# bioinformatics-centre/kaiju

Measured on AMD Instinct MI355X. Metric: classified reads/sec (150 bp), higher is better.
Workload: dtype u64

## Files before the change

kaiju_amd/csrc/capi.hip:

```cpp
#include <hip/hip_runtime.h>
#include <fcntl.h>
#include <sys/stat.h>
#include <time.h>
#include <unistd.h>

#include <algorithm>
#include <atomic>
#include <cstdio>
#include <cstring>
#include <future>
#include <memory>
#include <mutex>
#include <stdexcept>
#include <string>
#include <thread>
#include <vector>
#include <chrono>

#include "../../include/kaiju_gpu.h"
#include "fmi_stream.h"
#include "host_index.h"
#include "host_tables.h"
#include "kj_core.h"
#include "taxonomy.h"
// ... 203 lines not shown
  {
    const bool td = need || later;
    const uint64_t m = __ballot(td);
    if (m) {
      const uint32_t leader = (uint32_t)__builtin_ctzll(m);
      uint32_t base = 0;
      if (lane == leader) base = atomicAdd(todocount, (uint32_t)__popcll(m));
      base = (uint32_t)__shfl((int)base, (int)leader, 64);
      if (td) todo[base + (uint32_t)__popcll(m & ((1ull << lane) - 1ull))] = r;
    }
  }
}
template <bool LCA>
__global__ void __launch_bounds__(256)
k_mem_post2(DevIndex ix, Params p, Batch b, DevTaxonomy t, CompactHit *__restrict__ compact, const uint32_t *__restrict__ todo,
            const uint32_t *__restrict__ todocount) {
  const uint32_t n = *todocount;
  for (uint32_t i = blockIdx.x * 256 + threadIdx.x; i < n; i += gridDim.x * 256) {
    const uint32_t r = todo[i];
    Hit *h = b.hits + r;
    if (!mem_locate_read<false>(ix, p, h, kLocDeferRows)) mem_locate_read<false, true>(ix, p, h);
    if (LCA) compact[r] = compact_hit(t, *h);
  }
}

__global__ void __launch_bounds__(kFragBlock)
k_fragments_protein(const ConstTables *__restrict__ g_ct, Params p, SegTables st, Batch b, SegQueue sq, uint32_t *err) {
  __shared__ ConstTables s_ct;
  __shared__ int32_t s_entg[17];
  __shared__ uint8_t s_code[256];
  if (threadIdx.x < 17) s_entg[threadIdx.x] = st.ent_g32[threadIdx.x];
  {
    const uint32_t *src = reinterpret_cast<const uint32_t *>(g_ct);
    uint32_t *dst = reinterpret_cast<uint32_t *>(&s_ct);
    for (uint32_t i = threadIdx.x; i < sizeof(ConstTables) / 4; i += kFragBlock) dst[i] = src[i];
    for (uint32_t i = threadIdx.x; i < 256; i += kFragBlock) s_code[i] = 0;
    __syncthreads();
    if (threadIdx.x < 20) protein_code_entry(s_ct, threadIdx.x, s_code);
    __syncthreads();
  }
  const uint32_t r = blockIdx.x * kFragBlock + threadIdx.x;
  if (r >= b.n_reads) return;
  uint32_t e = 0;
  build_fragments_protein(s_ct, s_code, p, TrigCtx{s_entg, st.ent_locut32}, b, sq, r, &e);
  if (e) atomicOr(err, e);
}

struct CoopWave {
  uint64_t *prefix = nullptr;
  __device__ __forceinline__ uint64_t *pref() const { return prefix; }
  __device__ __forceinline__ void sync() const { __syncthreads(); }
  __device__ __forceinline__ int lane() const { return (int)(threadIdx.x & 63u); }
  __device__ __forceinline__ int width() const { return 64; }
  __device__ __forceinline__ void reduce_min(double &prob, int &t) const {
#pragma unroll
    for (int o = 32; o > 0; o >>= 1) {
      const double op = __shfl_xor(prob, o, 64);
      const int ot = __shfl_xor(t, o, 64);
      if (op < prob || (op == prob && ot < t)) { prob = op; t = ot; }
    }
  }
};

template <int T>
struct CoopTeam {
  uint64_t *prefix = nullptr;
  __device__ __forceinline__ uint64_t *pref() const { return prefix; }
  __device__ __forceinline__ void sync() const { __builtin_amdgcn_fence(__ATOMIC_ACQ_REL, "workgroup"); __builtin_amdgcn_wave_barrier(); }
  __device__ __forceinline__ int lane() const { return (int)(threadIdx.x & (uint32_t)(T - 1)); }
  __device__ __forceinline__ int width() const { return T; }
  __device__ __forceinline__ void reduce_min(double &prob, int &t) const {
#pragma unroll
    for (int o = T / 2; o > 0; o >>= 1) {
      const double op = __shfl_xor(prob, o, 64);
      const int ot = __shfl_xor(t, o, 64);
      if (op < prob || (op == prob && ot < t)) { prob = op; t = ot; }
    }
  }
};

constexpr int kSegBlock = 64, kSegStage = 2048;
__global__ void __launch_bounds__(kSegBlock)
k_seg(Params p, SegTables st, Batch b, SegQueue sq) {
  __shared__ int64_t s_entg[13];
  __shared__ double s_lnf[kSegLnf];
  __shared__ __attribute__((aligned(16))) uint8_t s_frag[kSegStage];
  __shared__ int32_t s_work[4 * kSegMaxRegions];
  __shared__ uint8_t s_cls[kSegStage];
  if (threadIdx.x < 13) s_entg[threadIdx.x] = st.ent_g[threadIdx.x];
  if (threadIdx.x < kSegLnf) s_lnf[threadIdx.x] = st.lnfact[threadIdx.x];
  __syncthreads();
  const SegCtx cx = seg_ctx(st, s_entg, s_lnf);
  __shared__ uint64_t s_pref[2 * (kSegPacked + 1)];
  CoopWave coop;
  coop.prefix = s_pref;
  const uint32_t n = min(*sq.count, sq.cap);
  for (uint32_t s = blockIdx.x; s < n; s += gridDim.x)
    seg_compute(cx, coop, b, p, sq, s, s_frag, kSegStage, s_work, s_cls, [] { __syncthreads(); });
}
#ifndef KJ_SEG_WAVES
#define KJ_SEG_WAVES 3
#endif
template <int T>
__global__ void __launch_bounds__(kSegBlock, KJ_SEG_WAVES)
k_seg_teams(Params p, SegTables st, Batch b, SegQueue sq) {
  constexpr int NT = kSegBlock / T, kStage = kSegStage / NT;
  __shared__ int64_t s_entg[13];
  __shared__ double s_lnf[kSegLnf];
  __shared__ __attribute__((aligned(16))) uint8_t s_frag[kSegStage];
  __shared__ int32_t s_work[NT * 4 * kSegMaxRegions];
  __shared__ uint8_t s_cls[kSegStage];
  if (threadIdx.x < 13) s_entg[threadIdx.x] = st.ent_g[threadIdx.x];
  if (threadIdx.x < kSegLnf) s_lnf[threadIdx.x] = st.lnfact[threadIdx.x];
  __syncthreads();
  const SegCtx cx = seg_ctx(st, s_entg, s_lnf);
  __shared__ uint64_t s_pref[NT * 2 * (kSegPacked + 1)];
  const uint32_t team = threadIdx.x / (uint32_t)T;
  CoopTeam<T> coop;
  coop.prefix = s_pref + team * 2 * (kSegPacked + 1);
  const uint32_t n = min(*sq.count, sq.cap);
  for (uint32_t s0 = blockIdx.x * NT; s0 < n; s0 += gridDim.x * NT) {
    const uint32_t s = s0 + team;
    if (s < n)
      seg_compute(cx, coop, b, p, sq, s, s_frag + team * kStage, kStage, s_work + team * 4 * kSegMaxRegions, s_cls + team * kStage,
                  [] { __builtin_amdgcn_fence(__ATOMIC_ACQ_REL, "workgroup"); __builtin_amdgcn_wave_barrier(); });
  }
}

__global__ void __launch_bounds__(kBlock)
k_seg_apply(const ConstTables *__restrict__ g_ct, Params p, Batch b, SegQueue sq, uint32_t *err) {
  __shared__ ConstTables s_ct;
  load_tables(s_ct, g_ct);
  const uint32_t r = blockIdx.x * kBlock + threadIdx.x;
  if (r >= b.n_reads) return;
  uint32_t e = 0;
  seg_apply_mem(s_ct, p, b, sq, r, &e);
  if (e) atomicOr(err, e);
}

template <class P>
__device__ __forceinline__ void mem_body(const DevIndex &ix, const Params &p, const Batch &b, const WorkList &wl,
                                         SIEntry *si_all, uint32_t si_cap, const VerboseOut &vb) {
  __shared__ __attribute__((aligned(16))) uint8_t s_win[kBlock * kWinStride];
  const uint64_t lane = (uint64_t)blockIdx.x * kBlock + threadIdx.x;
  LaneScratch ls;
  ls.si = si_all + lane * si_cap;
  ls.si_cap = si_cap;
  ls.win = s_win + threadIdx.x * kWinStride;
  mem_lane<P>(ix, p, b, wl, ls, vb);
}
#ifndef KJ_MEM_WAVES
#define KJ_MEM_WAVES 4
#endif
#ifdef KJ_PROF
__global__ void __launch_bounds__(kBlock, 3)
#else
__global__ void __launch_bounds__(kBlock, KJ_MEM_WAVES)
#endif
k_mem(DevIndex ix, Params p, Batch b, WorkList wl, SIEntry *si_all, uint32_t si_cap) {
  __shared__ __attribute__((aligned(16))) uint8_t s_win[kBlock * kWinStride];
  const uint64_t lane = (uint64_t)blockIdx.x * kBlock + threadIdx.x;
  LaneScratch ls;
  ls.si = si_all + lane * si_cap;
  ls.si_cap = si_cap;
  ls.win = s_win + threadIdx.x * kWinStride;
#ifdef KJ_PROF
  __shared__ unsigned long long s_prof[kBlock / 64][2 + 3 * PM_N];
  for (int x = threadIdx.x & 63; x < 2 + 3 * PM_N; x += 64) s_prof[threadIdx.x >> 6][x] = 0;
  ls.prof = s_prof[threadIdx.x >> 6];
  if ((threadIdx.x & 63) == 0) { ls.prof[0] = __builtin_readcyclecounter(); ls.prof[1] = PM_HEAD; }
#endif
  mem_lane2<false>(ix, p, b, wl, ls);
}
template <bool WIDE>
__global__ void __launch_bounds__(256)
k_mem_locate(DevIndex ix, Params p, Batch b, uint32_t *list, uint32_t *count) {
  const uint32_t r = blockIdx.x * 256 + threadIdx.x;
  const bool defer = r < b.n_reads && !mem_locate_read<WIDE>(ix, p, b.hits + r, list ? kLocDeferRows : 0u);
  const uint64_t m = __ballot(defer);
// ... 1292 lines not shown
  KJ_HIP(hipMemcpy(host_out, static_cast<const uint8_t *>(a.p) + offset_bytes, n_bytes, hipMemcpyDeviceToHost));
  return KAIJU_GPU_OK;
  });
}

struct kaiju_gpu_taxonomy {
  int device = 0;
  DevTaxonomy dev{};
  std::vector<void *> allocs;
  ~kaiju_gpu_taxonomy() {
    (void)hipSetDevice(device);
    for (void *p : allocs) (void)hipFree(p);
  }
};

__global__ void __launch_bounds__(256)
k_lca(DevTaxonomy t, const Hit *__restrict__ hits, uint32_t n, CompactHit *__restrict__ out) {
  const uint32_t r = blockIdx.x * 256 + threadIdx.x;
  if (r >= n) return;
  out[r] = compact_hit(t, hits[r]);
}

struct DevBuf {
  void *p = nullptr;
  size_t cap = 0;
};

struct kaiju_gpu_ctx {
  const kaiju_gpu_index *ix = nullptr;
  kaiju_gpu_params params{};
  Params kp{};
  hipStream_t stream = nullptr;
  hipEvent_t ev[6] = {nullptr, nullptr, nullptr, nullptr, nullptr, nullptr};
  bool ev_valid = false;
  int n_cu = 0, blocks_main = 0, blocks_retry = 0;
  DevBuf pep, frags, meta, counters, retry_list, seg_items, seg_recs;
  DevBuf scratch_main[10], scratch_retry[5], h_compact;
  DevBuf redo_bitmap, redo_list, redo_items, redo_index, redo_pool, redo_work, redo_cls;
  bool greedy2 = false;
  bool greedy3 = false;
  uint32_t g3_split = 1;
  uint32_t g3_threads = 512;
  uint32_t g1_pool = 192, g1_match = 64;
  bool g1_pool_set = false;
  uint32_t greedy_gate = 1u | 32u << 8;
  bool verbose = false;
  bool exact_pass = true;
  bool count_ops = false;
  bool mem_v1 = false;
  bool verbose_v1 = false;
  bool stage1_old = false;
  bool stage1_lane = false;
  bool lazy_seg = true;
  DevBuf seglist, loc_list, todo_list;
  int seg_team = 64;
  bool fused_post = true;
  const char *dump_frags = nullptr;
  uint32_t vb_text_cap = 0;
  DevBuf vb_nacc, vb_acc, vb_tlen, vb_text, vb_bestv, vb_bestv_retry;
  DevBuf vb_packed, vb_pos;
  std::vector<uint8_t> vb_host;
  std::vector<uint32_t> vb_h_nacc, vb_h_acc;
  DevBuf h_seqs, h_off, h_hits;
  kj_ingest_scratch *ingest = nullptr;
  DevBuf ing_text1, ing_text2, ing_names, ing_info;
  kj_format_scratch *format = nullptr;
  DevBuf fmt_pw, fmt_out, fmt_info;
  bool fmt_pw_ok = false;
  kaiju_gpu_stats stats{};
  uint32_t last_n = 0;
  uint32_t max_read_len = 1024;
  ~kaiju_gpu_ctx() {
    if (!ix) return;
    (void)hipSetDevice(ix->device);
    if (ingest) kj_ingest_free(ingest);
    if (format && kj_format_free) kj_format_free(format);
    DevBuf *all[] = {&fmt_pw, &fmt_out, &fmt_info, &ing_text1, &ing_text2, &ing_names, &ing_info, &pep, &frags, &meta, &counters, &retry_list, &seg_items, &seg_recs, &h_seqs, &h_off, &h_hits, &h_compact, &seglist, &loc_list, &todo_list,
                     &vb_nacc, &vb_acc, &vb_tlen, &vb_text, &vb_bestv, &vb_bestv_retry, &vb_packed, &vb_pos,
                     &redo_bitmap, &redo_list, &redo_items, &redo_index, &redo_pool, &redo_work, &redo_cls};
    for (DevBuf *b : all) if (b->p) (void)hipFree(b->p);
    for (int i = 0; i < 10; i++) if (scratch_main[i].p) (void)hipFree(scratch_main[i].p);
    for (int i = 0; i < 5; i++) if (scratch_retry[i].p) (void)hipFree(scratch_retry[i].p);
    for (auto &e : ev) if (e) (void)hipEventDestroy(e);
    if (stream) (void)hipStreamDestroy(stream);
  }
};

static int ensure(DevBuf &b, size_t bytes) {
  if (bytes <= b.cap) return 0;
  if (b.p) { KJ_HIP(hipFree(b.p)); b.p = nullptr; b.cap = 0; }
  const size_t want = bytes + bytes / 8 + 256;
  KJ_HIP(hipMalloc(&b.p, want));
  b.cap = want;
  return 0;
}

extern "C" void kaiju_gpu_default_params(kaiju_gpu_params *p, int mode) {
  if (!p) return;
  p->mode = mode ? 1 : 0;
  p->min_fragment_length = 11;
  p->mismatches = 3;
  p->min_score = 65;
  p->seed_length = 7;
  p->seg = 1;
  p->use_evalue = mode ? 1 : 0;
  p->min_evalue = 0.01;
  p->max_matches_SI = 20;
  p->max_match_ids = 20;
  p->input_is_protein = 0;
}

extern "C" int kaiju_gpu_create(kaiju_gpu_ctx **out, const kaiju_gpu_index *ix, const kaiju_gpu_params *p) {
  return guarded([&]() -> int {
  if (!out || !ix || !p) return fail(KAIJU_GPU_ERR_ARG, "NULL argument");
  *out = nullptr;
  if (p->mode != 0 && p->mode != 1) return fail(KAIJU_GPU_ERR_ARG, "mode must be 0 (MEM) or 1 (GREEDY)");
  if (p->min_fragment_length < 1 || p->min_fragment_length > 10000)
    return fail(KAIJU_GPU_ERR_UNSUPPORTED, "min_fragment_length out of range");
  if (p->mode == 1 && p->mismatches > (uint32_t)kMaxMismatch)
    return fail(KAIJU_GPU_ERR_UNSUPPORTED, "more than 8 mismatches are not supported");
  if (p->mode == 1 && p->seed_length < 1) return fail(KAIJU_GPU_ERR_ARG, "seed_length must be >= 1");
  if (p->max_match_ids > 20 || p->max_matches_SI > 64 || p->max_matches_SI < 1)
    return fail(KAIJU_GPU_ERR_UNSUPPORTED, "max_match_ids <= 20 and 1 <= max_matches_SI <= 64 required");
  std::unique_ptr<kaiju_gpu_ctx> c(new kaiju_gpu_ctx());
  c->ix = ix;
  c->params = *p;
  c->kp.mode = p->mode; c->kp.m = p->min_fragment_length; c->kp.mismatches = p->mismatches;
  c->kp.min_score = p->min_score; c->kp.seed_length = p->seed_length; c->kp.seg = p->seg ? 1 : 0;
  c->kp.max_matches_SI = p->max_matches_SI; c->kp.max_match_ids = p->max_match_ids;
  if (const char *e = getenv("KAIJU_GPU_DEBUG")) c->kp.debug = (uint32_t)atoi(e);
  if (const char *e = getenv("KAIJU_GPU_EXACT_PASS")) c->exact_pass = atoi(e) != 0;
  if (const char *e = getenv("KAIJU_GPU_MEM_LANE")) c->mem_v1 = !strcmp(e, "v1");
  if (const char *e = getenv("KAIJU_GPU_VERBOSE_LANE")) c->verbose_v1 = !strcmp(e, "v1");
  c->dump_frags = getenv("KAIJU_GPU_DUMP_FRAGS");
  if (const char *e = getenv("KAIJU_GPU_STAGE1")) { c->stage1_old = !strcmp(e, "old"); c->stage1_lane = !strcmp(e, "lane"); }
  if (const char *e = getenv("KAIJU_GPU_LAZY_SEG")) c->lazy_seg = atoi(e) != 0;
  if (const char *e = getenv("KAIJU_GPU_FUSED_POST")) c->fused_post = atoi(e) != 0;
  if (const char *e = getenv("KAIJU_GPU_SEG_TEAM")) { const int v = atoi(e); if (v == 8 || v == 16 || v == 32 || v == 64) c->seg_team = v; }
  if (ix->id_mode == KAIJU_GPU_IDS_SEQUENCE && p->mode == 0) c->kp.flags |= kParamXOrder;
  if (p->input_is_protein) c->kp.flags |= kParamProtein;
  KJ_HIP(hipSetDevice(ix->device));
  hipDeviceProp_t prop;
  KJ_HIP(hipGetDeviceProperties(&prop, ix->device));
  c->n_cu = prop.multiProcessorCount;
  int occ = 0;
  if (p->mode == 0) KJ_HIP(hipOccupancyMaxActiveBlocksPerMultiprocessor(&occ, k_mem, kBlock, 0));
  else {
    const bool g_wide = ix->dev.mb_base != nullptr;
    const uint32_t g_k = g_wide ? ix->dev.kmer_k : ix->dev.kline_k;
    c->greedy2 = ix->dev.blocks64 && (g_wide ? ix->dev.kmer64 != nullptr : ix->dev.kline != nullptr) && g_k >= 2 &&
                 g_k <= p->seed_length && p->seed_length >= 3;
    if (const char *e = getenv("KAIJU_GPU_GREEDY_LANE")) { if (!strcmp(e, "v1")) c->greedy2 = false; }
#ifdef KJ_GREEDY3
    if (const char *e = getenv("KAIJU_GPU_GREEDY_LANE")) { if (!strcmp(e, "v3")) c->greedy3 = c->greedy2 && !g_wide; }
    if (const char *e = getenv("KAIJU_GPU_G3_SPLIT")) c->g3_split = (uint32_t)atoi(e);
    if (const char *e = getenv("KAIJU_GPU_G3_THREADS")) { const int v = atoi(e); if (v >= 64 && v <= kG3Threads && v % 64 == 0) c->g3_threads = (uint32_t)v; }
#else
    if (const char *e = getenv("KAIJU_GPU_GREEDY_LANE")) {
      if (!strcmp(e, "v3")) return fail(KAIJU_GPU_ERR_UNSUPPORTED, "KAIJU_GPU_GREEDY_LANE=v3: this library was built without -DKJ_GREEDY3 (tests/tools/mem_variants.sh, variant g3)");
    }
#endif
    if (const char *e = getenv("KAIJU_GPU_GREEDY_GATE")) { int v = atoi(e); if (v == 0 || v == 1 || v == 3 || v == 7 || v == 15) c->greedy_gate = (c->greedy_gate & ~0xffu) | (uint32_t)v; }
    if (const char *e = getenv("KAIJU_GPU_GREEDY_WAITERS")) { int v = atoi(e); if (v >= 0 && v <= 64) c->greedy_gate = (c->greedy_gate & 0xffu) | (uint32_t)v << 8; }
    if (c->greedy2) {
      KJ_HIP(hipFuncSetAttribute(reinterpret_cast<const void *>(k_greedy2), hipFuncAttributeMaxDynamicSharedMemorySize,
                                 (int)kGreedy2Lds));
      KJ_HIP(hipFuncSetAttribute(reinterpret_cast<const void *>(k_greedy2_count), hipFuncAttributeMaxDynamicSharedMemorySize,
                                 (int)kGreedy2Lds));
      KJ_HIP(hipFuncSetAttribute(reinterpret_cast<const void *>(k_greedy2_wide), hipFuncAttributeMaxDynamicSharedMemorySize,
                                 (int)kGreedy2Lds));
      KJ_HIP(hipFuncSetAttribute(reinterpret_cast<const void *>(k_greedy2_wide_count), hipFuncAttributeMaxDynamicSharedMemorySize,
                                 (int)kGreedy2Lds));
      KJ_HIP(hipFuncSetAttribute(reinterpret_cast<const void *>(k_greedy2_vb), hipFuncAttributeMaxDynamicSharedMemorySize, (int)kGreedy2Lds));
      KJ_HIP(hipFuncSetAttribute(reinterpret_cast<const void *>(k_greedy2_wide_vb), hipFuncAttributeMaxDynamicSharedMemorySize, (int)kGreedy2Lds));
      if (g_wide) KJ_HIP(hipOccupancyMaxActiveBlocksPerMultiprocessor(&occ, k_greedy2_wide, kBlock, kGreedy2Lds));
      else KJ_HIP(hipOccupancyMaxActiveBlocksPerMultiprocessor(&occ, k_greedy2, kBlock, kGreedy2Lds));
    } else KJ_HIP(hipOccupancyMaxActiveBlocksPerMultiprocessor(&occ, k_greedy, kBlock, 0));
  }
  if (occ < 1) occ = 1;
  if (occ > 8) occ = 8;
  if (const char *e = getenv("KAIJU_GPU_BLOCKS_PER_CU")) { int v = atoi(e); if (v >= 1 && v <= 8) occ = v; }
  c->blocks_main = c->n_cu * occ;
  c->blocks_retry = p->mode == 0 ? 16 : 4;
  if (const char *e = getenv("KAIJU_GPU_G1_POOL")) { int v = atoi(e); if (v >= 64 && v <= 65535) { c->g1_pool = (uint32_t)v; c->g1_pool_set = true; } }
  if (const char *e = getenv("KAIJU_GPU_G1_MATCH")) { int v = atoi(e); if (v >= 16 && v <= 65535) c->g1_match = (uint32_t)v; }
  if (const char *e = getenv("KAIJU_GPU_RETRY_BLOCKS")) { int v = atoi(e); if (v >= 1 && v <= 256) c->blocks_retry = v; }
  KJ_HIP(hipStreamCreateWithFlags(&c->stream, hipStreamNonBlocking));
  for (auto &e : c->ev) KJ_HIP(hipEventCreate(&e));
  {
// ... 167 lines not shown
    if ((rc = ensure(c->scratch_main[0], lanes_main * si_cap * sizeof(SIEntry)))) return rc;
    const uint32_t si_cap_retry = (uint32_t)std::min<uint64_t>(2 * max_pair + 64, 1u << 24);
    int blocks_retry = c->blocks_retry;
    while (blocks_retry > 1 && (uint64_t)blocks_retry * kBlock * si_cap_retry * sizeof(SIEntry) > (1ull << 30)) blocks_retry /= 2;
    if ((rc = ensure(c->scratch_retry[0], (uint64_t)blocks_retry * kBlock * si_cap_retry * sizeof(SIEntry)))) return rc;
    if (n > 0) {
      const bool xo = (p.flags & kParamXOrder) != 0;
      SIEntry *si_main = static_cast<SIEntry *>(c->scratch_main[0].p);
      auto launch_v2 = [&](const Params &pp, const WorkList &wl, bool counting, bool second = false) {
        if (c->verbose) {
          if (mem_narrow2) hipLaunchKernelGGL(k_mem_vb, dim3(c->blocks_main), blk, 0, s, ix->dev, pp, b, wl, si_main, si_cap, vb.acc);
          else hipLaunchKernelGGL(k_mem_wide2_vb, dim3(c->blocks_main), blk, 0, s, ix->dev, pp, b, wl, si_main, si_cap, vb.acc);
        } else
        if (mem_narrow2) {
          if (second && !xo) hipLaunchKernelGGL(k_mem_second, dim3(c->blocks_main), blk, 0, s, ix->dev, pp, b, wl, si_main, si_cap);
          else if (counting) hipLaunchKernelGGL(k_mem_count, dim3(c->blocks_main), blk, 0, s, ix->dev, pp, b, wl, si_main, si_cap);
          else if (xo) hipLaunchKernelGGL(k_mem_x, dim3(c->blocks_main), blk, 0, s, ix->dev, pp, b, wl, si_main, si_cap);
          else hipLaunchKernelGGL(k_mem, dim3(c->blocks_main), blk, 0, s, ix->dev, pp, b, wl, si_main, si_cap);
        } else {
          if (counting) hipLaunchKernelGGL(k_mem_wide2_count, dim3(c->blocks_main), blk, 0, s, ix->dev, pp, b, wl, si_main, si_cap);
          else if (xo) hipLaunchKernelGGL(k_mem_wide2_x, dim3(c->blocks_main), blk, 0, s, ix->dev, pp, b, wl, si_main, si_cap);
          else hipLaunchKernelGGL(k_mem_wide2, dim3(c->blocks_main), blk, 0, s, ix->dev, pp, b, wl, si_main, si_cap);
        }
      };
      const bool defer = mem_v2;
      Params pd = p;
      if (defer) pd.flags |= kParamDeferLocate;
      if (mem_v2) {
        Params pm = pd;
        if (lazy) pm.flags |= kParamLazySeg;
        launch_v2(pm, wl_main, c->count_ops);
      } else if (!ix->dev.mb_base)
        hipLaunchKernelGGL(k_mem_v1, dim3(c->blocks_main), blk, 0, s, ix->dev, p, b, wl_main, si_main, si_cap, vb);
      else
        hipLaunchKernelGGL(k_mem_wide, dim3(c->blocks_main), blk, 0, s, ix->dev, p, b, wl_main, si_main, si_cap, vb);
      KJ_HIP(hipGetLastError());
      KJ_HIP(hipEventRecord(c->ev[3], s));
      uint32_t *todo = nullptr;
      const DevTaxonomy dt = tax ? tax->dev : DevTaxonomy{};
      CompactHit *const cmp = reinterpret_cast<CompactHit *>(d_compact);
      if (fused) {
        if ((rc = ensure(c->seglist, (size_t)n * 4 + 16))) return rc;
        if ((rc = ensure(c->todo_list, (size_t)n * 4 + 16))) return rc;
        todo = static_cast<uint32_t *>(c->todo_list.p);
        uint32_t *seglist = static_cast<uint32_t *>(c->seglist.p);
        if (tax) hipLaunchKernelGGL(k_mem_post1<true>, grid_reads, dim3(256), 0, s, ix->d_s1, ix->dev, p, b, dt, cmp, lazy ? 1 : 0, seglist, cnt + 22, todo, cnt + 26);
        else hipLaunchKernelGGL(k_mem_post1<false>, grid_reads, dim3(256), 0, s, ix->d_s1, ix->dev, p, b, dt, cmp, lazy ? 1 : 0, seglist, cnt + 22, todo, cnt + 26);
        KJ_HIP(hipGetLastError());
      }
      if (lazy) {
        if ((rc = ensure(c->seglist, (size_t)n * 4 + 16))) return rc;
        uint32_t *seglist = static_cast<uint32_t *>(c->seglist.p);
        if (!fused) hipLaunchKernelGGL(k_trigcheck, grid_reads, dim3(256), 0, s, ix->d_s1, p, b, seglist, cnt + 22);
        hipLaunchKernelGGL(k_segflag, dim3(c->n_cu * 4), dim3(256), 0, s, p, ix->st, b, sq, seglist, cnt + 22, cnt + 3);
        launch_seg(c, s, p, ix->st, b, sq);
        hipLaunchKernelGGL(k_seg_apply_list, dim3(c->n_cu * 4), blk, 0, s, ix->d_ct, p, b, sq, seglist, cnt + 22, cnt + 3);
        WorkList wl_seg;
        wl_seg.counter = cnt + 23; wl_seg.reads = seglist; wl_seg.n_items_ptr = cnt + 22; wl_seg.n_items = 0;
        wl_seg.retry_list = wl_main.retry_list; wl_seg.retry_count = wl_main.retry_count;
        launch_v2(pd, wl_seg, false, true);
        KJ_HIP(hipGetLastError());
      }
      hipLaunchKernelGGL(k_mem_retry, dim3(blocks_retry), blk, 0, s, ix->dev, p, b, wl_retry,
                         static_cast<SIEntry *>(c->scratch_retry[0].p), si_cap_retry, vb);
      KJ_HIP(hipGetLastError());
      if (defer && c->verbose) {
        if (mem_narrow2) hipLaunchKernelGGL(k_mem_verbose<false>, grid_reads, dim3(256), 0, s, ix->dev, p, b, vb);
        else hipLaunchKernelGGL(k_mem_verbose<true>, grid_reads, dim3(256), 0, s, ix->dev, p, b, vb);
        KJ_HIP(hipGetLastError());
      }
      if (defer && !fused) {
        if (mem_narrow2 && ix->dev.row_tax) {
          hipLaunchKernelGGL(k_mem_locate<false>, grid_reads, dim3(256), 0, s, ix->dev, p, b, loc_list, cnt + 24);
          hipLaunchKernelGGL(k_mem_locate_list<false>, dim3(c->n_cu * 8), dim3(256), 0, s, ix->dev, p, b, loc_list, cnt + 24);
        }
        else if (mem_narrow2) hipLaunchKernelGGL(k_mem_locate_team, grid_team, dim3(256), 0, s, ix->dev, p, b);
        else if (ix->dev.row_tax) {
          hipLaunchKernelGGL(k_mem_locate<true>, grid_reads, dim3(256), 0, s, ix->dev, p, b, loc_list, cnt + 24);
          hipLaunchKernelGGL(k_mem_locate_list<true>, dim3(c->n_cu * 8), dim3(256), 0, s, ix->dev, p, b, loc_list, cnt + 24);
        }
        else hipLaunchKernelGGL(k_mem_locate_wide, grid_team, dim3(256), 0, s, ix->dev, p, b);
        KJ_HIP(hipGetLastError());
      }
      if (exact_pass) {
        xp.si = static_cast<SIEntry *>(c->scratch_retry[0].p); xp.si_cap = si_cap_retry; xp.blocks_search = blocks_retry;
        xp.vb = vb;
        KJ_HIP(kj_launch_exact_pass(xp));
      }
      if (fused) {
        if (tax) hipLaunchKernelGGL(k_mem_post2<true>, dim3(c->n_cu * 8), dim3(256), 0, s, ix->dev, p, b, dt, cmp, todo, cnt + 26);
        else hipLaunchKernelGGL(k_mem_post2<false>, dim3(c->n_cu * 8), dim3(256), 0, s, ix->dev, p, b, dt, cmp, todo, cnt + 26);
        KJ_HIP(hipGetLastError());
      }
    } else KJ_HIP(hipEventRecord(c->ev[3], s));
  } else {
    const uint32_t frag_max = max_read_len / 3 + 4;
    GreedyArrays ga;
    ga.pool_cap = (c->verbose && !c->g1_pool_set) ? std::max<uint32_t>(c->g1_pool, 512u) : c->g1_pool; ga.match_cap = c->g1_match;
    const bool vb_g2 = c->verbose && !c->verbose_v1 && max_read_len / 3 + 4 < 65536;
    const bool use_g2 = c->greedy2 && (!c->verbose || vb_g2);
    const bool use_g3 = use_g2 && c->greedy3 && !c->verbose;
#ifdef KJ_GREEDY3
    const uint64_t lanes_g2 = use_g3 ? (uint64_t)c->n_cu * kG3Pool : lanes_main;
#else
    const uint64_t lanes_g2 = lanes_main;
#endif
    if (!use_g2) {
      if ((rc = ensure(c->scratch_main[0], lanes_main * ga.pool_cap * sizeof(GItem)))) return rc;
      if ((rc = ensure(c->scratch_main[1], lanes_main * ga.pool_cap * sizeof(uint16_t)))) return rc;
// ... 838 lines not shown
```

kaiju_amd/csrc/kj_core.h:

```cpp
#pragma once
#include <type_traits>
#include <stdint.h>

#if defined(__HIPCC__)
#include <hip/hip_runtime.h>
#define KJ_HD __host__ __device__ __forceinline__
#define KJ_HD_NOINLINE __host__ __device__ __noinline__
#else
#define KJ_HD inline
#define KJ_HD_NOINLINE inline
struct uint2 { uint32_t x, y; };
struct ulonglong2 { uint64_t x, y; };
#endif

namespace kj {

struct u128 { uint64_t x, y; };
typedef u128 u128_unaligned __attribute__((aligned(1)));
typedef uint32_t u32_unaligned __attribute__((aligned(1)));
typedef uint64_t u64_unaligned __attribute__((aligned(1)));

constexpr int kMaxIds = 21;
constexpr int kSbShift = 16;
constexpr uint32_t kHitIdCap = 1u, kHitSiCap = 2u;
// ... 373 lines not shown
  for (uint64_t step = 0; step <= n; step++) {
    if (tpos5 && (k & tvm) == 0) put_tpos5(tpos5, k >> tv_shift, g);
    if (row_tax) row_tax[k] = dense;
    const uint32_t c = symbol_at(ix, k);
    if (text) text[g - 1] = (uint8_t)c;
    if (c == 0) return;
    k = rank_c(ix, c, k);
    g--;
  }
}

KJ_HD uint32_t kmer_index(uint32_t idx, uint32_t c) { return idx * 20u + (c - 1u); }
KJ_HD void kmer_lookup(const DevIndex &ix, uint32_t idx, uint64_t &lo, uint64_t &hi) {
  if (ix.kmer32) { const uint2 e = ix.kmer32[idx]; lo = e.x; hi = (uint64_t)e.x + e.y; }
  else { const ulonglong2 e = ix.kmer64[idx]; lo = e.x; hi = e.x + e.y; }
}

KJ_HD uint32_t codon_fwd(const ConstTables &t, const uint8_t *s) {
  const uint32_t a = t.nuc[s[0]], b = t.nuc[s[1]], c = t.nuc[s[2]];
  if ((a | b | c) > 3u) return 255u;
  return t.codon_aa[a * 16 + b * 4 + c];
}
KJ_HD uint32_t codon_rev(const ConstTables &t, const uint8_t *s) {
  const uint32_t a = t.nuc[s[2]], b = t.nuc[s[1]], c = t.nuc[s[0]];
  if ((a | b | c) > 3u) return 255u;
  return t.codon_aa[(3 - a) * 16 + (3 - b) * 4 + (3 - c)];
}

constexpr int kSegWindow = 12, kSegDown = 5, kSegUp = 7, kSegMaxTrim = 50;
constexpr int kSegMaxRegions = 32;
constexpr int kSegPacked = 63;
constexpr int kSegLnf = 64;

#define KJ_SL(s, i) ((uint32_t)(s)[(i)] - 1u)

struct SegCtx {
  const int64_t *ent_g;
  int64_t ent_locut, ent_hicut;
  const double *lnf;
  const double *lnfact;
  uint32_t lnfact_n;
};
KJ_HD SegCtx seg_ctx(const SegTables &st, const int64_t *ent_g, const double *lnf) {
  SegCtx c; c.ent_g = ent_g; c.ent_locut = st.ent_locut; c.ent_hicut = st.ent_hicut;
  c.lnf = lnf; c.lnfact = st.lnfact; c.lnfact_n = st.lnfact_n;
  return c;
}

struct CoopSerial {
  uint64_t *prefix = nullptr;
  KJ_HD int lane() const { return 0; }
  KJ_HD int width() const { return 1; }
  KJ_HD void reduce_min(double &, int &) const {}
  KJ_HD uint64_t *pref() const { return prefix; }
  KJ_HD void sync() const {}
};

struct SegWin {
  uint64_t c0, c1;
  int64_t score;
};
KJ_HD void segwin_add(SegWin &w, const SegCtx &cx, uint32_t a, int d) {
  const uint32_t old = a < 16 ? (uint32_t)(w.c0 >> (4 * a)) & 15u : (uint32_t)(w.c1 >> (4 * (a - 16))) & 15u;
  w.score += cx.ent_g[(int)old + d] - cx.ent_g[old];
  if (a < 16) w.c0 += (uint64_t)(int64_t)d << (4 * a);
  else w.c1 += (uint64_t)(int64_t)d << (4 * (a - 16));
}
template <class S>
KJ_HD void segwin_open(SegWin &w, const SegCtx &cx, const S &s, int start) {
  w.c0 = w.c1 = 0; w.score = 0;
  for (int i = 0; i < kSegWindow; i++) segwin_add(w, cx, KJ_SL(s, start + i), +1);
}
template <class S>
KJ_HD void segwin_shift(SegWin &w, const SegCtx &cx, const S &s, int start) {
  segwin_add(w, cx, KJ_SL(s, start), -1);
  segwin_add(w, cx, KJ_SL(s, start + kSegWindow), +1);
}

KJ_HD double kj_lnfact(const SegCtx &cx, int n) {
  if (n < kSegLnf) return cx.lnf[n];
  return cx.lnfact[(uint32_t)n < cx.lnfact_n ? n : cx.lnfact_n - 1];
}

KJ_HD double seg_finish_prob(double ans1, double ans2, int total) {
  const double totseq = ((double)total) * 2.9957322735539909;
#if defined(__HIP_DEVICE_COMPILE__)
  return __dsub_rn(__dadd_rn(ans1, ans2), totseq);
#else
  volatile double t = ans1 + ans2;
  return t - totseq;
#endif
}

KJ_HD int zero_fields6(uint64_t x) {
  const uint64_t LOW5 = 0x7DF7DF7DF7DF7DFull;
  const uint64_t HI = 0x820820820820820ull;
  const uint64_t nzmask = (((x & LOW5) + LOW5) | x) & HI;
  return 10 - (int)popc64(nzmask);
}

KJ_HD double seg_prob_of_counts(const SegCtx &cx, uint64_t c0, uint64_t c1, int l);
KJ_HD double seg_window_prob_packed(const SegCtx &cx, const uint8_t *s, int l, int i) {
  uint64_t c0 = 0, c1 = 0;
  for (int k = 0; k < l; k++) {
    const uint32_t a = KJ_SL(s, i + k);
    if (a < 10) c0 += 1ull << (6 * a); else c1 += 1ull << (6 * (a - 10));
// ... 117 lines not shown
      while (loi - 1 >= lowlim && (cls[loi - 1 - first] & 2)) loi--;
      while (hii + 1 <= last && (cls[hii + 1 - first] & 2)) hii++;
    } else {
      if (wi + 1 == i) segwin_shift(w, cx, s, wi - first);
      else if (wi != i) segwin_open(w, cx, s, i - first);
      wi = i;
      if (w.score > cx.ent_locut) continue;
      {
        SegWin b;
        while (loi - 1 >= lowlim) {
          segwin_open(b, cx, s, loi - 1 - first);
          if (b.score > cx.ent_hicut) break;
          loi--;
        }
      }
      {
        SegWin f = w;
        while (hii + 1 <= last) {
          segwin_shift(f, cx, s, hii - first);
          if (f.score > cx.ent_hicut) break;
          hii++;
        }
      }
    }
    const int rawleft = loi - kSegDown, rawright = hii + kSegUp - 1;
    int tl, tr;
    seg_trim(cx, coop, s + rawleft, rawright - rawleft + 1, tl, tr);
    const int leftend = rawleft + tl, rightend = rawleft + tr;
    if constexpr (TOP) {
      if (i + kSegUp - 1 < leftend) {
        int32_t tb[1], te[1];
        bool ov = false;
        const int k = seg_scan<false>(cx, coop, s + rawleft, leftend - rawleft, offset + rawleft, tb, te, 0, 1, ov,
                                      cls ? cls + rawleft : nullptr);
        if (k > 0) {
          if (n < cap) { beg[n] = tb[0]; end[n] = te[0]; n++; } else overflow = true;
        }
      }
    }
    if constexpr (TOP) {
      if (n < cap) { beg[n] = leftend + offset; end[n] = rightend + offset; n++; } else overflow = true;
    } else {
      beg[0] = leftend + offset; end[0] = rightend + offset; n = 1;
    }
    i = hii < rightend + kSegDown ? hii : rightend + kSegDown;
    lowlim = i + 1;
  }
  return n;
}

template <class Coop, class Sync>
KJ_HD int seg_regions(const SegCtx &cx, const Coop &coop, const uint8_t *s, int len,
                      int32_t *left, int32_t *right, bool &overflow, int32_t *work, uint8_t *cls, Sync &&team_sync,
                      int cap = kSegMaxRegions) {
  int32_t *b = work, *e = work + cap;
  if (cls && len >= kSegWindow) {
    seg_classes(cx, coop, s, len, cls);
    team_sync();
  }
  const int n = seg_scan<true>(cx, coop, s, len, 0, b, e, 0, cap, overflow, cls);
  if (n == 0) return 0;
  int m = 0;
  int32_t cb = b[n - 1], ce = e[n - 1];
  for (int k = n - 2; k >= 0; k--) {
    if (cb - e[k] - 1 < 0) {
      if (ce < e[k]) ce = e[k];
      if (cb > b[k]) cb = b[k];
    } else {
      left[m] = cb; right[m] = ce; m++;
      cb = b[k]; ce = e[k];
    }
  }
  left[m] = cb; right[m] = ce; m++;
  for (int a = 0, z = m - 1; a < z; a++, z--) {
    int32_t t = left[a]; left[a] = left[z]; left[z] = t;
    t = right[a]; right[a] = right[z]; right[z] = t;
  }
  return m;
}

#if defined(__HIP_DEVICE_COMPILE__)
KJ_HD uint32_t fetch_work(uint32_t *counter) { return atomicAdd(counter, 1u); }
KJ_HD uint32_t append_slot(uint32_t *counter) { return atomicAdd(counter, 1u); }
#else
KJ_HD uint32_t fetch_work(uint32_t *counter) { return (*counter)++; }
KJ_HD uint32_t append_slot(uint32_t *counter) { return (*counter)++; }
#endif

struct PepBuf {
  uint8_t *base;
  uint32_t row;
  KJ_HD uint8_t get(uint32_t p) const { return base[(size_t)(p >> 2) * row + (p & 3u)]; }
  KJ_HD void put(uint32_t p, uint8_t v) const { base[(size_t)(p >> 2) * row + (p & 3u)] = v; }
  KJ_HD uint32_t get32(uint32_t p) const { return *reinterpret_cast<const uint32_t *>(base + (size_t)(p >> 2) * row); }
};
struct PepView {
  PepBuf b;
  uint32_t off;
  KJ_HD uint8_t operator[](int i) const { return b.get(off + (uint32_t)i); }
};

template <class S>
KJ_HD uint32_t diag_score(const ConstTables &t, const S &pep, uint32_t start, uint32_t len) {
  uint32_t s = 0;
  for (uint32_t i = 0; i < len; i++) { const uint32_t a = t.idx_to_aa[pep[start + i]]; s += (uint32_t)t.b62[a][a]; }
  return s;
}

KJ_HD void frag_insert(Frag *list, uint32_t &n, uint32_t cap, const Frag &f) {
// ... 206 lines not shown
    src = stage;
  }
  int32_t *left = work + 2 * kSegMaxRegions, *right = work + 3 * kSegMaxRegions;
  bool ov = false;
  const int n = seg_regions(cx, coop, src, (int)f.len, left, right, ov, work, (stage && f.len <= stage_cap) ? cls : nullptr, team_sync);
  if (coop.lane() != 0) return;
  SegRec rec;
  rec.overflow = (ov || n > kSegRecRegions || f.len > 65535u) ? 1 : 0;
  rec.n = (uint16_t)(n > kSegRecRegions ? kSegRecRegions : n);
  for (int k = 0; k < kSegRecRegions; k++) {
    rec.lr[k][0] = k < n ? (uint16_t)left[k] : 0;
    rec.lr[k][1] = k < n ? (uint16_t)right[k] : 0;
  }
  sq.recs[slot] = rec;
}

template <class Sink>
KJ_HD void seg_split(const ConstTables &t, const Params &p, const SegRec &rec, const uint8_t *pep,
                     const Frag &f, Sink &&sink) {
  const int nreg = rec.n;
  uint64_t start = 0;
  for (int r = 0; r <= nreg; r++) {
    const uint64_t length = (r < nreg ? (uint64_t)rec.lr[r][0] : (uint64_t)f.len) - start;
    if (length > p.m) {
      const uint64_t avail = start <= f.len ? f.len - start : 0;
      const uint32_t take = (uint32_t)(length < avail ? length : avail);
      Frag q; q.start = f.start + (uint32_t)start; q.len = take; q.flags = kFragChecked;
      if (p.mode == 1) {
        q.key = diag_score(t, pep, q.start, take);
        if (q.key >= p.min_score) sink(q);
      } else { q.key = (uint32_t)length; sink(q); }
    }
    if (r < nreg) start = (uint64_t)rec.lr[r][1] + 1;
  }
}
struct BigRegs { const int32_t *lr; int cnt; };
template <class Sink>
KJ_HD void seg_split_regs(const ConstTables &t, const Params &p, const BigRegs &regs, const uint8_t *pep,
                          const Frag &f, Sink &&sink) {
  const int nreg = regs.cnt;
  uint64_t start = 0;
  for (int r = 0; r <= nreg; r++) {
    const uint64_t length = (r < nreg ? (uint64_t)(uint32_t)regs.lr[2 * r] : (uint64_t)f.len) - start;
    if (length > p.m) {
      const uint64_t avail = start <= f.len ? f.len - start : 0;
      const uint32_t take = (uint32_t)(length < avail ? length : avail);
      Frag q; q.start = f.start + (uint32_t)start; q.len = take; q.flags = kFragChecked;
      if (p.mode == 1) {
        q.key = diag_score(t, pep, q.start, take);
        if (q.key >= p.min_score) sink(q);
      } else { q.key = (uint32_t)length; sink(q); }
    }
    if (r < nreg) start = (uint64_t)(uint32_t)regs.lr[2 * r + 1] + 1;
  }
}

struct BigSeg {
  uint2 *index;
  int32_t *lr;
  uint32_t *count;
  uint32_t cap;
};
constexpr uint32_t kBigSegLost = 0xffffffffu;
#if defined(__HIP_DEVICE_COMPILE__)
KJ_HD uint32_t append_many(uint32_t *counter, uint32_t n) { return atomicAdd(counter, n); }
#else
KJ_HD uint32_t append_many(uint32_t *counter, uint32_t n) { const uint32_t v = *counter; *counter += n; return v; }
#endif
template <class Coop, class Sync>
KJ_HD void seg_compute_big(const SegCtx &cx, const Coop &coop, const Batch &b, const SegQueue &sq, const BigSeg &big,
                           uint32_t slot, int32_t *work, int cap, uint8_t *cls, uint32_t *err_flags, Sync &&team_sync) {
  const SegWork wk = sq.items[slot];
  const ReadMeta rm = b.meta[wk.read];
  const Frag f = b.frags[rm.frag + wk.frag];
  const uint8_t *src = b.pep + rm.pep + f.start;
  int32_t *left = work + 2 * cap, *right = work + 3 * cap;
  bool ov = false;
  team_sync();
  const int n = seg_regions(cx, coop, src, (int)f.len, left, right, ov, work, cls, team_sync, cap);
  if (coop.lane() != 0) return;
  uint2 ent; ent.x = 0; ent.y = kBigSegLost;
  if (!ov) {
    const uint32_t off = append_many(big.count, (uint32_t)n);
    if ((uint64_t)off + (uint32_t)n <= big.cap) {
      for (int k = 0; k < n; k++) { big.lr[2 * ((size_t)off + k)] = left[k]; big.lr[2 * ((size_t)off + k) + 1] = right[k]; }
      ent.x = off; ent.y = (uint32_t)n;
    }
  }
  if (ent.y == kBigSegLost && err_flags) *err_flags |= 4u;
  big.index[slot] = ent;
}

struct FragAppend {
  Frag *dst; uint32_t *n; uint32_t cap;
  KJ_HD void operator()(const Frag &q) const { if (*n < cap) dst[(*n)++] = q; }
};

KJ_HD void build_fragments(const ConstTables &t, const Params &p, const TrigCtx &tc, const Batch &b,
                           const SegQueue &sq, uint32_t r, uint32_t *err_flags, uint8_t *stage, uint32_t stage_row,
                           uint32_t stage_words) {
  const uint64_t o0 = b.off[2 * (uint64_t)r], o1 = b.off[2 * (uint64_t)r + 1], o2 = b.off[2 * (uint64_t)r + 2];
  const uint32_t len1 = (uint32_t)(o1 - o0), len2 = (uint32_t)(o2 - o1);
  const uint32_t m3 = p.m * 3;
  Frag *list = b.frags + frag_base(b.off, r, p.m);
  const uint32_t cap = frag_cap(b.off, r, p.m);
  const uint64_t pbase = pep_base(b.off, r);
// ... 744 lines not shown
      uint32_t pos = k;
      while (pos > 0 && (list[pos - 1].key < f.key || (list[pos - 1].key == f.key && list[pos - 1].flags > f.flags))) {
        list[pos] = list[pos - 1]; pos--;
      }
      list[pos] = f;
    }
    for (uint32_t k = 0; k < n; k++) {
      uint32_t fl = 0;
      if (p.seg) {
        fl = kFragChecked;
        if (list[k].flags & 1u) {
          const uint32_t slot = append_slot(sq.count);
          if (slot >= sq.cap) { if (err_flags) *err_flags |= 2u; }
          else {
            SegWork wk; wk.read = r; wk.frag = k;
            sq.items[slot] = wk;
            pending = kNfragSegPending;
            fl = (slot + 1) << kFragSlotShift;
          }
        }
      }
      list[k].flags = fl;
    }
  }
  ReadMeta rm; rm.pep = pbase; rm.frag = (uint32_t)frag_base(b.off, r, p.m); rm.nfrag = n | pending;
  b.meta[r] = rm;
}

KJ_HD void seg_apply_mem(const ConstTables &t, const Params &p, const Batch &b, const SegQueue &sq, uint32_t r,
                         uint32_t *err_flags) {
  const ReadMeta rm = b.meta[r];
  const uint32_t raw = rm.nfrag;
  if (!(raw & kNfragSegPending)) return;
  const uint32_t n_orig = raw & ~kNfragSegPending;
  Frag *list = b.frags + rm.frag;
  const uint32_t cap = frag_cap(b.off, r, p.m);
  const uint8_t *pep = b.pep + rm.pep;
  uint32_t np = 0;
  for (uint32_t k = 0; k < n_orig; k++) {
    const Frag f = list[k];
    const uint32_t slot1 = f.flags >> kFragSlotShift;
    if (!slot1) continue;
    const SegRec rec = sq.recs[slot1 - 1];
    if (rec.overflow && err_flags) *err_flags |= 1u;
    uint32_t cnt = n_orig + np;
    seg_split(t, p, rec, pep, f, FragAppend{list, &cnt, cap});
    np = cnt - n_orig;
    list[k].flags |= kFragRemoved;
  }
  uint32_t w = 0;
  for (uint32_t k = 0; k < n_orig; k++) if (!(list[k].flags & kFragRemoved)) list[w++] = list[k];
  for (uint32_t q = 0; q < np; q++) { const Frag pc = list[n_orig + q]; frag_insert(list, w, cap, pc); }
  b.meta[r].nfrag = w;
}

KJ_HD void seg_apply_mem_big(const ConstTables &t, const Params &p, const Batch &b, const BigSeg &big, uint32_t r) {
  const ReadMeta rm = b.meta[r];
  const uint32_t raw = rm.nfrag;
  if (!(raw & kNfragSegPending)) return;
  const uint32_t n_orig = raw & ~kNfragSegPending;
  Frag *list = b.frags + rm.frag;
  const uint32_t cap = frag_cap(b.off, r, p.m);
  const uint8_t *pep = b.pep + rm.pep;
  uint32_t np = 0;
  for (uint32_t k = 0; k < n_orig; k++) {
    const Frag f = list[k];
    const uint32_t slot1 = f.flags >> kFragSlotShift;
    if (!slot1) continue;
    const uint2 ent = big.index[slot1 - 1];
    if (ent.y == kBigSegLost) continue;
    uint32_t cnt = n_orig + np;
    seg_split_regs(t, p, BigRegs{big.lr + 2 * (size_t)ent.x, (int)ent.y}, pep, f, FragAppend{list, &cnt, cap});
    np = cnt - n_orig;
    list[k].flags |= kFragRemoved;
  }
  uint32_t w = 0;
  for (uint32_t k = 0; k < n_orig; k++) if (!(list[k].flags & kFragRemoved)) list[w++] = list[k];
  for (uint32_t q = 0; q < np; q++) { const Frag pc = list[n_orig + q]; frag_insert(list, w, cap, pc); }
  b.meta[r].nfrag = w;
}

struct LaneWin {
  uint8_t *w;
  int32_t q;
};
KJ_HD void win_fill(LaneWin &lw, const uint8_t *fs, int flen, int top) {
  (void)flen;
  int q = top - (kWin - 1);
  if (q < 0) q = 0;
  lw.q = q;
  const u32_unaligned *src = reinterpret_cast<const u32_unaligned *>(fs + q);
  uint32_t *dst = reinterpret_cast<uint32_t *>(lw.w);
#pragma unroll
  for (int t = 0; t < kWin / 4; t++) dst[t] = src[t];
}
KJ_HD uint32_t win_get(LaneWin &lw, const uint8_t *fs, int flen, int pos) {
  if (pos < lw.q || pos >= lw.q + kWin) win_fill(lw, fs, flen, pos);
  return lw.w[pos - lw.q];
}

enum ProfSec : int { PS_HEAD, PS_AFTER_SEARCH, PS_VAR_NEXT, PS_VAR_MATCH, PS_EVAL_NEXT, PS_EVAL_MATCH, PS_POP, PS_POP_SEG, PS_FINISH,
                     PS_HANDOUT, PS_LOAD, PS_LOAD10, PS_STEP, PS_KMER, PS_LF1, PS_SA, PS_VM_RANK, PS_VM_PUSH, PS_META, PS_FRAG,
                     PS_FILL, PS_MLOAD, PS_END_MATCH, PS_START_J, PS_LOC_ROW, PS_TAIL, PS_N };
enum ProfSecM : int { PM_HEAD, PM_LOAD, PM_LOADFILL, PM_STEP, PM_KMER, PM_LF1, PM_SA, PM_META, PM_FRAG, PM_FILL, PM_TAIL, PM_END_MATCH,
                      PM_START_J, PM_NEXT_FRAG, PM_LOC_INIT, PM_LOC_NEXT_SI, PM_LOC_ROW, PM_FINISH, PM_N };
#if defined(KJ_PROF) && defined(__HIP_DEVICE_COMPILE__)
// ... 2671 lines not shown
```

Before: 472.6 million.

## Fuse SEG flag, compute and apply into one per-read block kernel

Adds a k_seg_read kernel that replaces the three-kernel sequence (segflag, seg compute, seg_apply_list) with a single launch where one wave per block handles one read. The read's fragments and peptide span are staged in LDS, window classes are computed once and reused for region finding, and fragments are split and reinserted in place. This removes two launches and the global round-trips of intermediate SEG state, at the cost of fewer active threads per read and serial lane-0 bookkeeping. It runs by default when the SEG team width is 64.

```diff
diff --git a/kaiju_amd/csrc/capi.hip b/kaiju_amd/csrc/capi.hip
--- a/kaiju_amd/csrc/capi.hip
+++ b/kaiju_amd/csrc/capi.hip
@@ -279,6 +279,7 @@
   __device__ __forceinline__ void sync() const { __syncthreads(); }
   __device__ __forceinline__ int lane() const { return (int)(threadIdx.x & 63u); }
   __device__ __forceinline__ int width() const { return 64; }
+  __device__ __forceinline__ bool any(bool v) const { return __ballot(v) != 0; }
   __device__ __forceinline__ void reduce_min(double &prob, int &t) const {
 #pragma unroll
     for (int o = 32; o > 0; o >>= 1) {
@@ -352,6 +353,31 @@
       seg_compute(cx, coop, b, p, sq, s, s_frag + team * kStage, kStage, s_work + team * 4 * kSegMaxRegions, s_cls + team * kStage,
                   [] { __builtin_amdgcn_fence(__ATOMIC_ACQ_REL, "workgroup"); __builtin_amdgcn_wave_barrier(); });
   }
+}
+
+__global__ void __launch_bounds__(kSegBlock, KJ_SEG_WAVES)
+k_seg_read(const ConstTables *__restrict__ g_ct, Params p, SegTables st, Batch b, SegQueue sq, const uint32_t *__restrict__ seglist,
+           const uint32_t *__restrict__ segcount, uint32_t *err) {
+  __shared__ int64_t s_entg[13];
+  __shared__ double s_lnf[kSegLnf];
+  __shared__ __attribute__((aligned(16))) uint8_t s_stage[kSegReadStage];
+  __shared__ __attribute__((aligned(16))) Frag s_list[kSegReadList];
+  __shared__ uint8_t s_cls[kSegReadStage];
+  __shared__ int32_t s_work[4 * kSegMaxRegions];
+  __shared__ uint32_t s_word[2];
+  __shared__ uint64_t s_pref[2 * (kSegPacked + 1)];
+  if (threadIdx.x < 13) s_entg[threadIdx.x] = st.ent_g[threadIdx.x];
+  if (threadIdx.x < kSegLnf) s_lnf[threadIdx.x] = st.lnfact[threadIdx.x];
+  __syncthreads();
+  const SegCtx cx = seg_ctx(st, s_entg, s_lnf);
+  CoopWave coop;
+  coop.prefix = s_pref;
+  const SegReadScratch sc{s_stage, s_cls, s_list, s_work, s_word};
+  const uint32_t n = *segcount;
+  uint32_t e = 0;
+  for (uint32_t i = blockIdx.x; i < n; i += gridDim.x)
+    seg_read(cx, coop, *g_ct, p, b, sq, seglist[i], &e, sc, [] { __syncthreads(); });
+  if (e) atomicOr(err, e);
 }
 
 __global__ void __launch_bounds__(kBlock)
@@ -1750,6 +1776,7 @@
   bool stage1_old = false;
   bool stage1_lane = false;
   bool lazy_seg = true;
+  bool lazy_seg_read = true;
   DevBuf seglist, loc_list, todo_list;
   int seg_team = 64;
   bool fused_post = true;
@@ -1833,6 +1860,7 @@
   c->dump_frags = getenv("KAIJU_GPU_DUMP_FRAGS");
   if (const char *e = getenv("KAIJU_GPU_STAGE1")) { c->stage1_old = !strcmp(e, "old"); c->stage1_lane = !strcmp(e, "lane"); }
   if (const char *e = getenv("KAIJU_GPU_LAZY_SEG")) c->lazy_seg = atoi(e) != 0;
+  if (const char *e = getenv("KAIJU_GPU_LAZY_SEG_READ")) c->lazy_seg_read = atoi(e) != 0;
   if (const char *e = getenv("KAIJU_GPU_FUSED_POST")) c->fused_post = atoi(e) != 0;
   if (const char *e = getenv("KAIJU_GPU_SEG_TEAM")) { const int v = atoi(e); if (v == 8 || v == 16 || v == 32 || v == 64) c->seg_team = v; }
   if (ix->id_mode == KAIJU_GPU_IDS_SEQUENCE && p->mode == 0) c->kp.flags |= kParamXOrder;
@@ -2106,9 +2134,13 @@
         if ((rc = ensure(c->seglist, (size_t)n * 4 + 16))) return rc;
         uint32_t *seglist = static_cast<uint32_t *>(c->seglist.p);
         if (!fused) hipLaunchKernelGGL(k_trigcheck, grid_reads, dim3(256), 0, s, ix->d_s1, p, b, seglist, cnt + 22);
-        hipLaunchKernelGGL(k_segflag, dim3(c->n_cu * 4), dim3(256), 0, s, p, ix->st, b, sq, seglist, cnt + 22, cnt + 3);
-        launch_seg(c, s, p, ix->st, b, sq);
-        hipLaunchKernelGGL(k_seg_apply_list, dim3(c->n_cu * 4), blk, 0, s, ix->d_ct, p, b, sq, seglist, cnt + 22, cnt + 3);
+        if (c->lazy_seg_read && c->seg_team == 64)
+          hipLaunchKernelGGL(k_seg_read, dim3(c->n_cu * 32), dim3(kSegBlock), 0, s, ix->d_ct, p, ix->st, b, sq, seglist, cnt + 22, cnt + 3);
+        else {
+          hipLaunchKernelGGL(k_segflag, dim3(c->n_cu * 4), dim3(256), 0, s, p, ix->st, b, sq, seglist, cnt + 22, cnt + 3);
+          launch_seg(c, s, p, ix->st, b, sq);
+          hipLaunchKernelGGL(k_seg_apply_list, dim3(c->n_cu * 4), blk, 0, s, ix->d_ct, p, b, sq, seglist, cnt + 22, cnt + 3);
+        }
         WorkList wl_seg;
         wl_seg.counter = cnt + 23; wl_seg.reads = seglist; wl_seg.n_items_ptr = cnt + 22; wl_seg.n_items = 0;
         wl_seg.retry_list = wl_main.retry_list; wl_seg.retry_count = wl_main.retry_count;
diff --git a/kaiju_amd/csrc/kj_core.h b/kaiju_amd/csrc/kj_core.h
--- a/kaiju_amd/csrc/kj_core.h
+++ b/kaiju_amd/csrc/kj_core.h
@@ -449,6 +449,7 @@
   KJ_HD int lane() const { return 0; }
   KJ_HD int width() const { return 1; }
   KJ_HD void reduce_min(double &, int &) const {}
+  KJ_HD bool any(bool v) const { return v; }
   KJ_HD uint64_t *pref() const { return prefix; }
   KJ_HD void sync() const {}
 };
@@ -672,9 +673,9 @@
 template <class Coop, class Sync>
 KJ_HD int seg_regions(const SegCtx &cx, const Coop &coop, const uint8_t *s, int len,
                       int32_t *left, int32_t *right, bool &overflow, int32_t *work, uint8_t *cls, Sync &&team_sync,
-                      int cap = kSegMaxRegions) {
+                      int cap = kSegMaxRegions, bool cls_ready = false) {
   int32_t *b = work, *e = work + cap;
-  if (cls && len >= kSegWindow) {
+  if (cls && len >= kSegWindow && !cls_ready) {
     seg_classes(cx, coop, s, len, cls);
     team_sync();
   }
@@ -987,6 +988,26 @@
       } else { q.key = (uint32_t)length; sink(q); }
     }
     if (r < nreg) start = (uint64_t)(uint32_t)regs.lr[2 * r + 1] + 1;
+  }
+}
+
+template <class Sink>
+KJ_HD void seg_split_lists(const ConstTables &t, const Params &p, const int32_t *left, const int32_t *right, int n,
+                           const uint8_t *pep, const Frag &f, Sink &&sink) {
+  const int nreg = n > kSegRecRegions ? kSegRecRegions : n;
+  uint64_t start = 0;
+  for (int r = 0; r <= nreg; r++) {
+    const uint64_t length = (r < nreg ? (uint64_t)(uint16_t)left[r] : (uint64_t)f.len) - start;
+    if (length > p.m) {
+      const uint64_t avail = start <= f.len ? f.len - start : 0;
+      const uint32_t take = (uint32_t)(length < avail ? length : avail);
+      Frag q; q.start = f.start + (uint32_t)start; q.len = take; q.flags = kFragChecked;
+      if (p.mode == 1) {
+        q.key = diag_score(t, pep, q.start, take);
+        if (q.key >= p.min_score) sink(q);
+      } else { q.key = (uint32_t)length; sink(q); }
+    }
+    if (r < nreg) start = (uint64_t)(uint16_t)right[r] + 1;
   }
 }
 
@@ -1837,6 +1858,136 @@
   for (uint32_t k = 0; k < n_orig; k++) if (!(list[k].flags & kFragRemoved)) list[w++] = list[k];
   for (uint32_t q = 0; q < np; q++) { const Frag pc = list[n_orig + q]; frag_insert(list, w, cap, pc); }
   b.meta[r].nfrag = w;
+}
+
+constexpr uint32_t kSegReadStage = 2u * 6u * 16u * (uint32_t)kS1UnitsLong;
+constexpr uint32_t kSegReadList = 208;
+struct SegReadScratch {
+  uint8_t *stage;
+  uint8_t *cls;
+  Frag *list;
+  int32_t *work;
+  uint32_t *word;
+};
+template <bool OWN, class Coop, class Sync>
+KJ_HD void seg_read_body(const SegCtx &cx, const Coop &coop, const ConstTables &t, const Params &p, const Batch &b,
+                         const SegQueue &sq, uint32_t r, const ReadMeta &rm, uint32_t nf, uint32_t cap, uint32_t lo,
+                         uint32_t span, uint32_t *err_flags, const SegReadScratch &sc, Sync &&team_sync) {
+  Frag *G = b.frags + rm.frag;
+  Frag *L = OWN ? sc.list : G;
+  const uint8_t *pep = b.pep + rm.pep;
+  const uint8_t *res = OWN ? sc.stage : pep;
+  const uint32_t off = OWN ? lo : 0u;
+  const uint32_t lane = (uint32_t)coop.lane(), width = (uint32_t)coop.width();
+  if (OWN) {
+    const u128 *src = reinterpret_cast<const u128 *>(pep + lo);
+    u128 *dst = reinterpret_cast<u128 *>(sc.stage);
+    for (uint32_t x = lane; x < span / 16; x += width) dst[x] = src[x];
+    team_sync();
+  }
+  uint32_t ntrig = 0;
+  for (uint32_t k = 0; k < nf; k++) {
+    const uint32_t fs = L[k].start, fl = L[k].len;
+    const uint8_t *s = res + (fs - off);
+    const int nwin = (int)fl - kSegWindow + 1;
+    bool hit = false;
+    for (int w = (int)lane; w < nwin; w += (int)width) {
+      SegWin sw{0, 0, 0};
+      segwin_open(sw, cx, s, w);
+      const uint8_t c = (uint8_t)((sw.score <= cx.ent_locut ? 1 : 0) | (sw.score <= cx.ent_hicut ? 2 : 0));
+      if (OWN) sc.cls[fs - off + (uint32_t)w] = c;
+      hit = hit || (c & 1);
+    }
+    const bool trig = coop.any(hit);
+    if (lane == 0) L[k].flags = trig ? 0u : kFragChecked;
+    ntrig += trig ? 1u : 0u;
+  }
+  if (ntrig && lane == 0) sc.word[0] = append_many(sq.count, ntrig);
+  team_sync();
+  uint32_t cnt = nf;
+  bool pending = false;
+  if (ntrig) {
+    uint32_t slot = sc.word[0];
+    int32_t *left = sc.work + 2 * kSegMaxRegions, *right = sc.work + 3 * kSegMaxRegions;
+    for (uint32_t k = 0; k < nf; k++) {
+      const Frag f = L[k];
+      if (f.flags != 0u) continue;
+      const uint32_t sl = slot++;
+      if (sl >= sq.cap) {
+        if (lane == 0) { if (err_flags) *err_flags |= 2u; L[k].flags = kFragChecked; }
+        continue;
+      }
+      bool ov = false;
+      const int n = seg_regions(cx, coop, res + (f.start - off), (int)f.len, left, right, ov, sc.work,
+                                OWN ? sc.cls + (f.start - off) : nullptr, team_sync, kSegMaxRegions, true);
+      if (lane == 0) {
+        SegWork wk; wk.read = r; wk.frag = k;
+        sq.items[sl] = wk;
+        SegRec rec;
+        rec.overflow = (ov || n > kSegRecRegions || f.len > 65535u) ? 1 : 0;
+        rec.n = (uint16_t)(n > kSegRecRegions ? kSegRecRegions : n);
+        for (int q = 0; q < kSegRecRegions; q++) {
+          rec.lr[q][0] = q < n ? (uint16_t)left[q] : 0;
+          rec.lr[q][1] = q < n ? (uint16_t)right[q] : 0;
+        }
+        sq.recs[sl] = rec;
+        if (rec.overflow && err_flags) *err_flags |= 1u;
+        seg_split_lists(t, p, left, right, n, pep, f, FragAppend{L, &cnt, cap});
+        L[k].flags = ((sl + 1) << kFragSlotShift) | kFragRemoved;
+      }
+      pending = true;
+      team_sync();
+    }
+  }
+  if (lane == 0) {
+    uint32_t w = nf;
+    if (pending) {
+      w = 0;
+      for (uint32_t k = 0; k < nf; k++) if (!(L[k].flags & kFragRemoved)) L[w++] = L[k];
+      for (uint32_t q = nf; q < cnt; q++) { const Frag pc = L[q]; frag_insert(L, w, cap, pc); }
+    }
+    b.meta[r].nfrag = w;
+    sc.word[1] = cnt;
+  }
+  if (OWN) {
+    team_sync();
+    const uint32_t total = sc.word[1];
+    for (uint32_t k = lane; k < total; k += width) G[k] = L[k];
+  }
+  uint64_t *h8 = reinterpret_cast<uint64_t *>(b.hits + r);
+  for (uint32_t x = lane; x < (uint32_t)(sizeof(Hit) / 8); x += width) h8[x] = 0;
+}
+template <class Coop, class Sync>
+KJ_HD void seg_read(const SegCtx &cx, const Coop &coop, const ConstTables &t, const Params &p, const Batch &b,
+                    const SegQueue &sq, uint32_t r, uint32_t *err_flags, const SegReadScratch &sc, Sync &&team_sync) {
+  const ReadMeta rm = b.meta[r];
+  const uint32_t nf = rm.nfrag & ~kNfragSegPending;
+  const uint32_t cap = frag_cap(b.off, r, p.m);
+  const uint32_t lane = (uint32_t)coop.lane(), width = (uint32_t)coop.width();
+  bool own = cap <= kSegReadList && nf <= cap;
+  uint32_t lo = 0, span = 0;
+  team_sync();
+  if (own) {
+    const Frag *G = b.frags + rm.frag;
+    for (uint32_t k = lane; k < nf; k += width) sc.list[k] = G[k];
+    team_sync();
+    uint32_t a = 0xffffffffu, z = 0;
+    for (uint32_t k = 0; k < nf; k++) {
+      const uint32_t fs = sc.list[k].start, fe = fs + sc.list[k].len;
+      if (fs < a) a = fs;
+      if (fe > z) z = fe;
+      if (fe < fs) z = 0xffffffffu;
+    }
+    if (nf) {
+      lo = a & ~15u;
+      const uint64_t sp = ((uint64_t)z - lo + 15u) & ~15ull;
+      own = sp <= kSegReadStage;
+      span = (uint32_t)sp;
+    }
+    if (((rm.pep + lo) & 15u) != 0 || (reinterpret_cast<uintptr_t>(b.pep) & 15u) != 0) own = false;
+  }
+  if (own) seg_read_body<true>(cx, coop, t, p, b, sq, r, rm, nf, cap, lo, span, err_flags, sc, team_sync);
+  else seg_read_body<false>(cx, coop, t, p, b, sq, r, rm, nf, cap, 0u, 0u, err_flags, sc, team_sync);
 }
 
 KJ_HD void seg_apply_mem_big(const ConstTables &t, const Params &p, const Batch &b, const BigSeg &big, uint32_t r) {
```

Result: slower. 452.3 million (-4.3%).
